# zitongbai/bipedal_control

Measured on AMD Instinct MI355X. Metric: MPC solves/s (H1, horizon=100), higher is better.
Workload: dtype f64; 1 GPU; Unitree H1 trot (template tiled from t = 0), horizon=100 intervals (dt 0.015), batch=256 per GPU perturbed initial states, cold start, 1 SQP iteration (BASELINE.json configs[1]); solver=sqp, global_batch=256, problems_on_rank0=256, shooting_nodes=108, nx=22, nu=22

## Files before the change

### bipedal_control_amd/csrc/k_node.hip

```cpp
#include <hip/hip_runtime.h>
#include <hip/hip_ext.h>

#include <stdexcept>

#include "kernel_launchers.h"
#include "launch.h"
#include "kernels/rollout.h"

namespace bpmpc {

template <int NJ>
__global__ __launch_bounds__(kWave) void k_prepare(Launch L) {
  constexpr int NX = 12 + NJ, NU = 12 + NJ;
  const int s = blockIdx.x, b = s / L.N, k = s % L.N;
  const int g = L.buf.p_grid[b];
  const int n = L.buf.g_nodes[g];
  if (k >= n) { if (threadIdx.x == 0) L.buf.n_info[s] = 0; return; }
  const size_t gs = (size_t)g * L.N + k;
  if (threadIdx.x == 0) L.buf.n_info[s] = 8 | ((L.buf.g_mode[gs] & 3) << 1) | (L.buf.g_kind[gs] == 1 ? 1 : 0);
  if (threadIdx.x < kNodeAux) {
    const int t = threadIdx.x;
    L.buf.n_aux[(size_t)s * kNodeAux + t] = t == 0 ? L.buf.g_dt[gs] : t < 5 ? L.buf.g_zref[gs * 4 + t - 1] : t < 9 ? L.buf.g_zdref[gs * 4 + t - 5] : 0.0;
  }
  prepare_node<NJ>(*L.model, L.buf.g_kind[gs], L.buf.g_mode[gs], L.buf.g_start[gs], L.cold != 0, k == n - 1, L.buf.p_tgt_n[b],
// ... 172 lines not shown
    u[(size_t)i * NU + l] = a * uff0 + (1.0 - a) * uff1 + kx;
  }
}

template <int NJ>
__global__ __launch_bounds__(kWave) void k_ls_begin(Launch L) {
  __shared__ double partial[3 * kWave + 5];
  linesearch_begin<NJ>(partial, problem_ls<NJ>(L, blockIdx.x));
}

template <int NJ>
__global__ __launch_bounds__(kWave) void k_trial(Launch L) {
  constexpr int NX = 12 + NJ, NU = 12 + NJ;
  __shared__ TrialWorkspace<NJ> ws;
  const int sidx = blockIdx.x, b = sidx / L.N, k = sidx % L.N;
  if (L.buf.done[b]) return;
  if (k >= L.buf.g_nodes[L.buf.p_grid[b]]) return;
  const NodeInputs in = node_inputs<NJ>(L, b, k);
  const double* dx = L.buf.dx + ((size_t)b * (L.N + 1) + k) * NX;
  trial_node<NJ>(*L.model, ws, in, L.buf.alpha[b], dx, L.buf.du + (size_t)sidx * NU, dx + NX, L.buf.trial_perf + (size_t)sidx * 3);
}

template <int NJ, bool CHAIN>
__global__ __launch_bounds__(kTrialWaves * kWave) __attribute__((amdgpu_waves_per_eu(3, 3)))
void k_trial_fast(Launch L) {
  using C = LinFastCfg<NJ, true, CHAIN>;
  constexpr int NX = 12 + NJ, NU = 12 + NJ, LPN = C::LPN, NPW = C::NPW;
  __shared__ LinFastNodeLds<NJ, false, CHAIN> lds[kTrialWaves * NPW];
  __shared__ LinFastShared<NJ, false> shared;
  const int sub = threadIdx.x / LPN, g = threadIdx.x % LPN;
  const int widx = blockIdx.x * (kTrialWaves * NPW) + sub;
  {
    const int total = L.batch * L.klen, w0 = blockIdx.x * (kTrialWaves * NPW), w1 = (w0 + kTrialWaves * NPW < total ? w0 + kTrialWaves * NPW : total) - 1;
    bool any = false;
    for (int pb = w0 / L.klen; pb <= w1 / L.klen; ++pb) any = any || L.buf.done[pb] == 0;
    if (!any) return;
  }
  bool valid = widx < L.batch * L.klen;
  const int b = valid ? widx / L.klen : 0, k = valid ? L.k0 + widx % L.klen : 0;
  const double* dx = L.buf.dx + ((size_t)b * (L.N + 1) + k) * NX;
  {
    const int fin = L.buf.done[b];
    const double alpha = L.buf.alpha[b];
    const int info = L.buf.n_info[(size_t)b * L.N + k];
    const size_t s0 = (size_t)b * L.N + k;
    const double* xk = L.buf.x + ((size_t)b * (L.N + 1) + k) * NX;
    const TrialPre pre = trial_preload<C>(xk, xk + NX, L.buf.u + s0 * NU, L.buf.xref + s0 * NX, dx, dx + NX, L.buf.du + s0 * NU, g, L.buf.n_aux + s0 * kNodeAux);
    load_shared_model<kTrialWaves * kWave>(*L.model, shared, threadIdx.x);
    NodeInputs in;
    in.kind = info & 1; in.mode = (info >> 1) & 3; in.dt = 0.0;
    in.x = xk; in.xnext = xk + NX; in.u = L.buf.u + s0 * NU; in.xref = L.buf.xref + s0 * NX; in.zref = nullptr; in.zdref = nullptr;
    __syncthreads();
    valid = valid && fin == 0 && info != 0;
    const size_t s = valid ? s0 : 0;
    trial_fast<NJ, C>(*L.model, shared, lds[sub], valid, in, alpha, dx, L.buf.du + s * NU, dx + NX, L.buf.trial_perf + s * 3, g, nullptr, &pre);
  }
}

template <int NJ, bool CHAIN>
__global__ __launch_bounds__(kTrialWaves * kWave) void k_constraint_values(Launch L, double* eqv) {
  using C = LinFastCfg<NJ, true, CHAIN>;
  constexpr int NX = 12 + NJ, NU = 12 + NJ, LPN = C::LPN, NPW = C::NPW;
  __shared__ LinFastNodeLds<NJ, false, CHAIN> lds[kTrialWaves * NPW];
  __shared__ LinFastShared<NJ, false> shared;
  load_shared_model<kTrialWaves * kWave>(*L.model, shared, threadIdx.x);
  __syncthreads();
  const int sub = threadIdx.x / LPN, g = threadIdx.x % LPN;
  const int widx = blockIdx.x * (kTrialWaves * NPW) + sub;
  bool valid = widx < L.batch * L.klen;
  const int b = valid ? widx / L.klen : 0, k = valid ? L.k0 + widx % L.klen : 0;
  const int grid = L.buf.p_grid[b];
  valid = valid && k < L.buf.g_nodes[grid] && L.buf.g_kind[(size_t)grid * L.N + k] == 0;
  const size_t s = valid ? (size_t)b * L.N + k : 0;
  const NodeInputs in = node_inputs<NJ>(L, b, k);
  const double* dx = L.buf.dx + ((size_t)b * (L.N + 1) + k) * NX;
  double perf[3];
  trial_fast<NJ, C, true>(*L.model, shared, lds[sub], valid, in, 0.0, dx, L.buf.du + s * NU, dx + NX, perf, g, eqv + s * kMaxEqRows);
}

template <int NJ, bool CHAIN>
__global__ __launch_bounds__(kWave) void k_rollout(const DeviceModel* model, RolloutArgs a) {
  __shared__ RolloutLds<NJ, CHAIN> w;
  load_shared_model<kWave>(*model, w.shared, threadIdx.x);
  __syncthreads();
  rollout_policy<NJ, CHAIN>(*model, w, a);
}

constexpr int kDecideThreads = 256;
template <int NJ>
__global__ __launch_bounds__(kDecideThreads) void k_ls_decide(Launch L, int look_first) {
  __shared__ double partial[3 * kDecideThreads + 5];
  linesearch_decide<NJ, kDecideThreads>(partial, problem_ls<NJ>(L, blockIdx.x), L.ls, look_first != 0);
}

constexpr int kTailThreads = 512;
template <int NJ, bool CHAIN>
__global__ __launch_bounds__(kTailThreads) void k_ls_tail(Launch L, int first_round, int max_trials, int pending) {
  using C = LinFastCfg<NJ, true, CHAIN>;
  constexpr int NX = 12 + NJ, NU = 12 + NJ, LPN = C::LPN, NPW = C::NPW, CHUNK = (kTailThreads / kWave) * NPW;
  const int b = blockIdx.x;
  if (L.buf.done[b]) return;
  __shared__ LinFastNodeLds<NJ, false, CHAIN> lds[CHUNK];
  __shared__ LinFastShared<NJ, false> shared;
  __shared__ double partial[3 * kTailThreads + 5];
  volatile const int* done = L.buf.done + b;
  volatile const double* alpha = L.buf.alpha + b;
  if (pending) {
    int bb = b;
    asm volatile("" : "+s"(bb));
    linesearch_decide<NJ, kTailThreads, true>(partial, problem_ls<NJ>(L, bb), L.ls);
    __threadfence();
    __syncthreads();
    if (*done) return;
  }
  load_shared_model<kTailThreads>(*L.model, shared, threadIdx.x);
  __syncthreads();
  const int sub = threadIdx.x / LPN, g = threadIdx.x % LPN;
  const int n = L.buf.g_nodes[L.buf.p_grid[b]];
  for (int round = first_round; round < max_trials; ++round) {
    const double al = *alpha;
    for (int k0 = 0; k0 < n; k0 += CHUNK) {
      const int k = k0 + sub;
      const bool valid = k < n;
      const int kk = valid ? k : 0;
      const size_t s = (size_t)b * L.N + kk;
      const NodeInputs in = node_inputs<NJ>(L, b, kk);
      const double* dx = L.buf.dx + ((size_t)b * (L.N + 1) + kk) * NX;
      unsigned opaque = 0;
      asm volatile("" : "+v"(opaque));
      const auto& sh = *reinterpret_cast<const LinFastShared<NJ, false>*>(reinterpret_cast<const char*>(&shared) + opaque);
      trial_fast<NJ, C>(*L.model, sh, lds[sub], valid, in, al, dx, L.buf.du + s * NU, dx + NX, L.buf.trial_perf + s * 3, g);
    }
    __threadfence();
    __syncthreads();
    int bb = b;
    asm volatile("" : "+s"(bb));
    const ProblemLS p = problem_ls<NJ>(L, bb);
    linesearch_decide<NJ, kTailThreads, false>(partial, p, L.ls);
    __threadfence();
    __syncthreads();
    if (*done) break;
  }
}

__global__ __launch_bounds__(256) void k_copy_pairs(const double* a_src, double* a_dst, size_t na, const double* b_src, double* b_dst, size_t nb,
                                                     int* iterations, int* active, int batch) {
  const size_t i0 = (size_t)blockIdx.x * blockDim.x + threadIdx.x, stride = (size_t)gridDim.x * blockDim.x;
  const double2* a2 = reinterpret_cast<const double2*>(a_src);
  const double2* b2 = reinterpret_cast<const double2*>(b_src);
  double2* ad = reinterpret_cast<double2*>(a_dst);
  double2* bd = reinterpret_cast<double2*>(b_dst);
  for (size_t i = i0; i < na / 2; i += stride) ad[i] = a2[i];
  for (size_t i = i0; i < nb / 2; i += stride) bd[i] = b2[i];
  if (i0 == 0) { if (na & 1) a_dst[na - 1] = a_src[na - 1]; if (nb & 1) b_dst[nb - 1] = b_src[nb - 1]; }
  if (iterations) for (size_t i = i0; i < (size_t)batch; i += stride) { iterations[i] = 0; active[i] = 1; }
}

namespace kl {

void prepare(int nj, int slots, hipStream_t st, const Launch& L) { KL_NJ(nj, hipLaunchKernelGGL(k_prepare<NJ>, dim3(slots), dim3(kWave), 0, st, L)); }
void linearize_reference(int nj, int slots, hipStream_t st, const Launch& L) { KL_NJ(nj, hipLaunchKernelGGL(k_linearize<NJ>, dim3(slots), dim3(kWave), 0, st, L)); }
// ... 15 lines not shown
      else launch(k_linearize_fast<NJ, false, true>);
    } else {
      if (materialise) launch(k_linearize_fast<NJ, true, false>);
      else launch(k_linearize_fast<NJ, false, false>);
    }
  });
}
void warm_shift(int nj, int slots, hipStream_t st, const Launch& L, const int* restarted) {
  KL_NJ(nj, hipLaunchKernelGGL(k_warm_shift<NJ>, dim3(slots), dim3(kWave), 0, st, L, restarted));
}
void ls_begin(int nj, int batch, hipStream_t st, const Launch& L) { KL_NJ(nj, hipLaunchKernelGGL(k_ls_begin<NJ>, dim3(batch), dim3(kWave), 0, st, L)); }
void trial_reference(int nj, int slots, hipStream_t st, const Launch& L) { KL_NJ(nj, hipLaunchKernelGGL(k_trial<NJ>, dim3(slots), dim3(kWave), 0, st, L)); }
int trial_fast_workgroups(int nj, int nodes) {
  const int per_wg = kTrialWaves * (nj == 10 ? LinFastCfg<10, true>::NPW : LinFastCfg<12, true>::NPW);
  return (nodes + per_wg - 1) / per_wg;
}
void trial_fast(int nj, int nodes, hipStream_t st, const Launch& L) {
  const int grid = trial_fast_workgroups(nj, nodes);
  KL_NJ(nj, {
    if (L.serial_legs) hipLaunchKernelGGL((k_trial_fast<NJ, true>), dim3(grid), dim3(kTrialWaves * kWave), 0, st, L);
    else hipLaunchKernelGGL((k_trial_fast<NJ, false>), dim3(grid), dim3(kTrialWaves * kWave), 0, st, L);
  });
}
void ls_decide(int nj, int batch, hipStream_t st, const Launch& L, bool look_first) { KL_NJ(nj, hipLaunchKernelGGL(k_ls_decide<NJ>, dim3(batch), dim3(kDecideThreads), 0, st, L, look_first ? 1 : 0)); }
void ls_tail(int nj, int batch, hipStream_t st, const Launch& L, int first_round, int max_trials, bool pending) {
  KL_NJ(nj, {
    if (L.serial_legs) hipLaunchKernelGGL((k_ls_tail<NJ, true>), dim3(batch), dim3(kTailThreads), 0, st, L, first_round, max_trials, pending ? 1 : 0);
    else hipLaunchKernelGGL((k_ls_tail<NJ, false>), dim3(batch), dim3(kTailThreads), 0, st, L, first_round, max_trials, pending ? 1 : 0);
  });
}
void constraint_values(int nj, int nodes, hipStream_t st, const Launch& L, double* eqv) {
  const int grid = trial_fast_workgroups(nj, nodes);
  KL_NJ(nj, {
    if (L.serial_legs) hipLaunchKernelGGL((k_constraint_values<NJ, true>), dim3(grid), dim3(kTrialWaves * kWave), 0, st, L, eqv);
    else hipLaunchKernelGGL((k_constraint_values<NJ, false>), dim3(grid), dim3(kTrialWaves * kWave), 0, st, L, eqv);
  });
}
void rollout(int nj, bool serial_legs, int batch, hipStream_t st, const DeviceModel* model, const RolloutArgs& a) {
  KL_NJ(nj, {
    constexpr bool kChainFits = LinFastCfg<NJ, false, true>::LPN == 16;
    const dim3 grid((batch + LinFastCfg<NJ>::NPW - 1) / LinFastCfg<NJ>::NPW);
    if constexpr (kChainFits) {
      if (serial_legs) { hipLaunchKernelGGL((k_rollout<NJ, true>), grid, dim3(kWave), 0, st, model, a); return; }
    }
    hipLaunchKernelGGL((k_rollout<NJ, false>), grid, dim3(kWave), 0, st, model, a);
  });
}
void copy_pairs(int grid, hipStream_t st, const double* a_src, double* a_dst, size_t na, const double* b_src, double* b_dst, size_t nb,
                int* iterations, int* active, int batch) {
  hipLaunchKernelGGL(k_copy_pairs, dim3(grid > 0 ? grid : 1), dim3(256), 0, st, a_src, a_dst, na, b_src, b_dst, nb, iterations, active, batch);
}
// ... 4 lines not shown
```

### bipedal_control_amd/csrc/kernel_launchers.h

```cpp
#pragma once
#include <hip/hip_runtime.h>

#include <cstddef>
#include <stdexcept>

namespace bpmpc {

#define KL_NJ(nj, ...)                                                          \
  do {                                                                          \
    if ((nj) == 10) { constexpr int NJ = 10; __VA_ARGS__; }                     \
    else if ((nj) == 12) { constexpr int NJ = 12; __VA_ARGS__; }                \
    else throw std::runtime_error("unsupported joint count");                   \
  } while (0)

struct Launch;
struct DeviceModel;
struct RolloutArgs;
struct DdpBuffers;
struct TickArgs;
struct TickCommandArgs;
struct RestartArgs;

namespace kl {

void prepare(int nj, int slots, hipStream_t st, const Launch& L);
void linearize_reference(int nj, int slots, hipStream_t st, const Launch& L);
void linearize_fast(int nj, bool materialise, int nodes, hipStream_t st, const Launch& L, hipEvent_t ev_start = nullptr, hipEvent_t ev_stop = nullptr);
void warm_shift(int nj, int slots, hipStream_t st, const Launch& L, const int* restarted = nullptr);
void ls_begin(int nj, int batch, hipStream_t st, const Launch& L);
void trial_reference(int nj, int slots, hipStream_t st, const Launch& L);
int trial_fast_workgroups(int nj, int nodes);
void trial_fast(int nj, int nodes, hipStream_t st, const Launch& L);
void ls_decide(int nj, int batch, hipStream_t st, const Launch& L, bool look_first = false);
void ls_tail(int nj, int batch, hipStream_t st, const Launch& L, int first_round, int max_trials, bool pending);
void constraint_values(int nj, int nodes, hipStream_t st, const Launch& L, double* eqv);
void rollout(int nj, bool serial_legs, int batch, hipStream_t st, const DeviceModel* model, const RolloutArgs& a);
void copy_pairs(int grid, hipStream_t st, const double* a_src, double* a_dst, size_t na, const double* b_src, double* b_dst, size_t nb,
                int* iterations, int* active, int batch);

void project_reference(int nj, int slots, hipStream_t st, const Launch& L);
void project_lu_s(int nj, int max_vel_rows, bool packed, int nodes, hipStream_t st, const Launch& L);
void project_fast(int nj, bool packed, bool joint_rows, int nodes, hipStream_t st, const Launch& L);

void riccati_reference(int nj, int batch, hipStream_t st, const Launch& L);
void riccati_fast(int nj, bool joint_rows, int batch, hipStream_t st, const Launch& L);
void riccati_fast8(int nj, bool joint_rows, int batch, hipStream_t st, const Launch& L);

void riccati_wave(int nj, bool two_per_simd, bool joint_rows, int batch, hipStream_t st, const Launch& L);
void riccati_rollout(int nj, int batch, hipStream_t st, const Launch& L);

void ddp_policy(int nj, int batch, hipStream_t st, const Launch& L, const DdpBuffers& d);
void ddp_cost(int nj, int batch, bool fast, hipStream_t st, const Launch& L, const DdpBuffers& d);
void ddp_select(int nj, int batch, hipStream_t st, const Launch& L, const DdpBuffers& d, double armijo);
void ddp_nominal(int nj, int batch, hipStream_t st, const Launch& L, const DdpBuffers& d);
void ddp_finish(int nj, int batch, hipStream_t st, const Launch& L, const DdpBuffers& d);
void ddp_keep_times(int batch, int N, hipStream_t st, const DdpBuffers& d, double* tp_time, int* tp_kind, int* tp_nodes, int* tp_grid);

// ... 7 lines not shown
```

### bipedal_control_amd/csrc/kernels/linesearch.h

```cpp
#pragma once
#include "node_lq.h"

namespace bpmpc {

constexpr int kMaxTargetPoints = 8;
constexpr int kStatsStride = 16;

struct LineSearchSettings {
  double g_max, g_min, alpha_decay, alpha_min, gamma_c, armijo_factor, delta_tol, cost_tol;
  int max_iterations;
};

template <int NJ>
BP_DEVICE void prepare_node(const DeviceModel& md, int kind, int mode, double t_start, bool cold, bool last, int n_pts, const double* tgt_t,
                            const double* tgt_x, const double* x0, double* xref, double* x, double* u, double* x_terminal) {
  constexpr int NX = 12 + NJ, NU = 12 + NJ;
  BP_LANES(tid, kWave) {
    if (tid < NX) {
      double val;
      if (n_pts == 1 || t_start <= tgt_t[0]) {
        val = tgt_x[tid];
      } else if (t_start >= tgt_t[n_pts - 1]) {
        val = tgt_x[(n_pts - 1) * NX + tid];
      } else {
// ... 16 lines not shown
struct TrialWorkspace {
  static constexpr int NX = 12 + NJ, NU = 12 + NJ;
  NodeWorkspace<NJ> node;
  double tx[NX], tu[NU], txn[NX];
};

template <int NJ>
BP_DEVICE void trial_node(const DeviceModel& md, TrialWorkspace<NJ>& ws, NodeInputs in, double alpha, const double* dx, const double* du,
                          const double* dxn, double* perf) {
  constexpr int NX = 12 + NJ, NU = 12 + NJ;
  BP_LANES(tid, kWave) {
    if (tid < NX) {
      ws.tx[tid] = in.x[tid] + alpha * dx[tid];
      ws.txn[tid] = in.xnext[tid] + alpha * dxn[tid];
    }
    if (tid < NU) ws.tu[tid] = (in.kind == 1) ? 0.0 : in.u[tid] + alpha * du[tid];
  }
  BP_SYNC();
  in.x = ws.tx;
  in.u = ws.tu;
  in.xnext = ws.txn;
  node_performance<NJ>(md, ws.node, in, perf);
}

struct ProblemLS {
  int n_nodes;
  const double* node_perf;
  const double* trial_perf;
  const double* x0;
  double *x, *u;
  const double *dx, *du;
  const double* summary;
  double* base;
  double* alpha;
  int* done;
  int* active;
  int* iterations;
  double* stats;
  int* remaining;
};

template <int NJ>
BP_DEVICE void linesearch_begin(double* partial , const ProblemLS& p) {
  constexpr int NX = 12 + NJ;
  BP_LANES(tid, kWave) {
    double a = 0.0, b = 0.0, c = 0.0;
    for (int k = tid; k < p.n_nodes; k += kWave) { a += p.node_perf[3 * k]; b += p.node_perf[3 * k + 1]; c += p.node_perf[3 * k + 2]; }
    if (tid < NX) { const double d = p.x0[tid] - p.x[tid]; b += d * d; }
    partial[tid] = a; partial[kWave + tid] = b; partial[2 * kWave + tid] = c;
  }
  BP_SYNC();
  BP_LANES(tid, kWave) {
    if (tid < 3) {
      double s = 0.0;
      for (int i = 0; i < kWave; ++i) s += partial[tid * kWave + i];
      partial[3 * kWave + 2 + tid] = s;
    }
  }
  BP_SYNC();
  BP_LANES(tid, kWave) {
    if (tid == 0) {
      const double a = partial[3 * kWave + 2], b = partial[3 * kWave + 3], c = partial[3 * kWave + 4];
// ... 102 lines not shown
  BP_SYNC();
  const bool accepted = partial[3 * NL] != 0.0;
  if (accepted) {
#if !defined(BPMPC_HOST_EMULATION)
#pragma unroll
    for (int j = 0; j < UPD; ++j) {
      const int idx = (int)threadIdx.x + j * NL;
      if (idx < nxe) p.x[idx] = xv[j] + alpha * dxv[j];
      if (idx < nue) p.u[idx] = uv[j] + alpha * duv[j];
    }
    int t0 = (int)threadIdx.x;
    if constexpr (!PRE) asm volatile("" : "+v"(t0));
    for (int idx = t0 + UPD * NL; idx < nxe; idx += NL) p.x[idx] += alpha * p.dx[idx];
    for (int idx = t0 + UPD * NL; idx < nue; idx += NL) p.u[idx] += alpha * p.du[idx];
#else
    BP_LANES(tid, NL) {
      for (int idx = tid; idx < (p.n_nodes + 1) * NX; idx += NL) p.x[idx] += alpha * p.dx[idx];
      for (int idx = tid; idx < p.n_nodes * NU; idx += NL) p.u[idx] += alpha * p.du[idx];
    }
#endif
  }
}

}
```

### bipedal_control_amd/csrc/kernels/riccati_fast.h

```cpp
#pragma once
#include <hip/hip_runtime.h>

#include "../device_model.h"
#include "riccati.h"
#include "project_node.h"
#include "linesearch.h"

namespace bpmpc {

struct RiccatiFastIO {
  RiccatiIO base;
  const double *Wt, *Qp, *Mt;
  const double* Vt;
  const double *lqA, *lqB, *lqb, *lqq, *lqr, *qrd, *gdt;
  const DeviceModel* model;
  const double* zero_one;
  const int* mode;
  double *Acl, *bcl;
  double *kff;
  double *mvec, *mscal;
  double* Kfull;
  double* prof;
  int k_lo, k_hi;
  double* carry;
// ... 18 lines not shown
  return __hiloint2double(hi, lo);
}
template <int NJ>
__device__ __forceinline__ void linesearch_begin_wave(double* partial , const ProblemLS& p, int lane) {
  constexpr int NX = 12 + NJ;
  {
    double a = 0.0, b = 0.0, c = 0.0;
    for (int k = lane; k < p.n_nodes; k += kWave) { a += p.node_perf[3 * k]; b += p.node_perf[3 * k + 1]; c += p.node_perf[3 * k + 2]; }
    if (lane < NX) { const double d = p.x0[lane] - p.x[lane]; b += d * d; }
    partial[lane] = a; partial[kWave + lane] = b; partial[2 * kWave + lane] = c;
  }
  lds_wave_sync();
  if (lane < 3) {
    double s = 0.0;
    for (int i = 0; i < kWave; ++i) s += partial[lane * kWave + i];
    partial[3 * kWave + 2 + lane] = s;
  }
  lds_wave_sync();
  if (lane == 0) {
    p.base[0] = partial[3 * kWave + 2]; p.base[1] = partial[3 * kWave + 3]; p.base[2] = partial[3 * kWave + 4];
    p.alpha[0] = 1.0;
    const bool run = p.active[0] != 0;
    p.done[0] = run ? 0 : 1;
    if (run) atomicAdd(p.remaining, 1);
  }
}
__device__ __forceinline__ double lds1(const double& r) {
  typedef const volatile __attribute__((address_space(3))) double* lds_cvp;
  return *(lds_cvp)(&r);
}
struct d2 { double x, y; };
__device__ __forceinline__ d2 lds_pair(const double* p) {
  const double2 v = *reinterpret_cast<const double2*>(p);
  return d2{v.x, v.y};
}

__device__ __forceinline__ double fast_reciprocal(double x) {
  double r = __builtin_amdgcn_rcp(x);
  double e = __builtin_fma(-x, r, 1.0);
  r = __builtin_fma(r, e, r);
  e = __builtin_fma(-x, r, 1.0);
  r = __builtin_fma(r, e, r);
  return r;
}

template <int ROWS>
// ... 305 lines not shown
```

### bipedal_control_amd/csrc/launch.h

```cpp
#pragma once
#include <hip/hip_runtime.h>

#include <cstddef>

#include "device_model.h"
#include "kernels/linesearch.h"
#include "kernels/node_lq.h"
#include "kernels/project_node.h"
#include "kernels/riccati_fast.h"
#include "kernels/linearize_fast.h"

namespace bpmpc {

struct Buffers {
  int *g_kind, *g_mode, *g_nodes;
  double *g_dt, *g_start, *g_zref, *g_zdref;
  int* p_grid;
  double *p_x0, *p_tgt_t, *p_tgt_x;
  int* p_tgt_n;
  double *x, *u, *x_init, *u_init, *xref;
  double *A, *B, *b, *Q, *R, *P, *q, *r, *c, *C, *D, *e, *perf;
  int* nc;
  double *Px, *Pu, *Pe, *At, *Bt, *bt, *Qt, *Rt, *Pt, *qt, *rt;
  double *Wt, *Qp, *Mt;
  double* Vt;
  int* nut;
  int* n_info;
  double* n_aux;
  double* lin_park;
  double* lin_dump;
  double* qrd;
  double *Kt, *kt, *dx, *du, *K, *summary, *dx0;
  double *Acl, *bcl, *kff, *mvec, *mscal, *rprof;
  double *x_prev, *u_prev, *K_prev, *tp_time;
  int *tp_kind, *tp_nodes, *tp_grid;
  double *roll_t, *roll_x0, *roll_x, *roll_u;
  int *roll_steps, *roll_status;
  double *g_time, *rg_t0, *rg_start, *p_t0, *p_cmd, *lib_d;
  int *rg_gait, *rg_status, *rg_rows, *lib_i;
  double* ric_carry;
  double* zero_page;
  double *trial_perf, *base, *alpha, *stats;
  int *done, *active, *iterations, *remaining;
};

struct DdpBuffers {
  int cap;
  int nv;
  double alpha_v[kMaxDdpSteps];
  double* lff;
  double *rec_t, *rec_x, *rec_u, *cost;
  int* rec_n;
  double *end_x, *end_u;
  int *roll_steps, *roll_status;
  double *sol_t, *sol_x, *sol_u;
  int* sol_n;
  double *merit0, *merit, *alpha, *update_is;
  int *accepted, *failed, *n_points;
};

constexpr int kLinMaxEvents = 8;
struct Launch {
  const DeviceModel* model;
  Buffers buf;
  int batch, N;
  int k0, klen;
// ... 45 lines not shown
}

template <int NJ>
__device__ __forceinline__ ProblemLS problem_ls(const Launch& L, int b) {
  constexpr int NX = 12 + NJ, NU = 12 + NJ;
  ProblemLS p;
  const size_t s0 = (size_t)b * L.N;
  p.n_nodes = L.buf.g_nodes[L.buf.p_grid[b]];
  p.node_perf = L.buf.perf + s0 * 3;
  p.trial_perf = L.buf.trial_perf + s0 * 3;
  p.x0 = L.buf.p_x0 + (size_t)b * NX;
  p.x = L.buf.x + (size_t)b * (L.N + 1) * NX;
  p.u = L.buf.u + s0 * NU;
  p.dx = L.buf.dx + (size_t)b * (L.N + 1) * NX;
  p.du = L.buf.du + s0 * NU;
  p.summary = L.buf.summary + (size_t)b * 4;
  p.base = L.buf.base + (size_t)b * 3;
  p.alpha = L.buf.alpha + b;
  p.done = L.buf.done + b;
  p.active = L.buf.active + b;
  p.iterations = L.buf.iterations + b;
  p.stats = L.buf.stats + (size_t)b * kStatsStride;
  p.remaining = L.buf.remaining;
  return p;
}

template <int NJ>
__device__ __forceinline__ bool riccati_fast_io(const Launch& L, RiccatiFastIO& io, double* lds_scratch ) {
  constexpr int NX = 12 + NJ, NU = 12 + NJ;
  const int b = blockIdx.x;
  const int tid_ = threadIdx.x;
  io.with_ls = L.k0 == 0;
  if (io.with_ls) io.ls = problem_ls<NJ>(L, b);
  if (!L.buf.active[b]) {
    if (io.with_ls && tid_ < kWave) linesearch_begin_wave<NJ>(lds_scratch, io.ls, tid_);
    return false;
  }
  const size_t s0 = (size_t)b * L.N;
  double* dx0 = L.buf.dx0 + (size_t)b * NX;
  if (tid_ < NX) dx0[tid_] = L.buf.p_x0[(size_t)b * NX + tid_] - L.buf.x[(size_t)b * (L.N + 1) * NX + tid_];
  __syncthreads();
  io.base.N = L.buf.g_nodes[L.buf.p_grid[b]];
  io.base.nut = L.buf.nut + s0;
  io.base.At = L.buf.At + s0 * NX * NX; io.base.Bt = L.buf.Bt + s0 * NX * NU; io.base.bt = L.buf.bt + s0 * NX;
  io.base.Qt = L.buf.Qt + s0 * NX * NX; io.base.Rt = L.buf.Rt + s0 * NU * NU; io.base.Pt = L.buf.Pt + s0 * NU * NX;
  io.base.qt = L.buf.qt + s0 * NX; io.base.rt = L.buf.rt + s0 * NU;
// ... 26 lines not shown
```

### bipedal_control_amd/csrc/solver.hip

```cpp
#include <hip/hip_runtime.h>

#include <cmath>
#include <cstdint>
#include <algorithm>
#include <cstring>
#include <map>
#include <tuple>
#include <memory>
#include <stdexcept>
#include <string>
#include <vector>

#include "solver.h"
#include "reference_gen.h"
#include "kernels/rollout.h"

#define TIMED_ON(on, cls, ...)                                                      \
  do {                                                                              \
    hipEvent_t ev_a_, ev_b_;                                                        \
    time_begin(cls, &ev_a_, &ev_b_, on);                                            \
    __VA_ARGS__;                                                                    \
    time_end(cls, ev_a_, ev_b_, on);                                                \
    HIP_CHECK(hipGetLastError());                                                   \
  } while (0)
// ... 38 lines not shown
  if (sweep_eight_waves()) { TIMED("riccati", kl::riccati_fast8(nj(), !sweep_completes_joint_rows(), batch, stream, L)); return; }
  if (!sweep_wave_regime()) {
    TIMED("riccati", kl::riccati_fast(nj(), !sweep_completes_joint_rows(), batch, stream, L));
    return;
  }
  TIMED("riccati", { kl::riccati_wave(nj(), sweep_two_per_simd(), !sweep_completes_joint_rows(), batch, stream, L); if (L.k0 == 0) kl::riccati_rollout(nj(), batch, stream, L); });
}
void bpmpc_solver::stage_riccati() {
  const Launch L = launch_params();
  if (settings.reference_kernels) TIMED("riccati", kl::riccati_reference(nj(), batch, stream, L));
  else launch_riccati(L);
}
void bpmpc_solver::stage_linesearch() {
  const Launch L = launch_params();
  if (settings.reference_kernels) HIP_CHECK(hipMemsetAsync(buf.remaining, 0, sizeof(int), stream));
  hipEvent_t ev_a, ev_b;
  time_begin("linesearch", &ev_a, &ev_b);
  if (settings.reference_kernels) kl::ls_begin(nj(), batch, stream, L);
  int max_trials = 0;
  for (double a = 1.0; a >= ls.alpha_min; a *= ls.alpha_decay) ++max_trials;
  if (!settings.reference_kernels) {
    const int nodes = batch * L.klen;
    static const int wide_rounds = [] { const char* e = std::getenv("BPMPC_LS_WIDE_ROUNDS"); const int v = e ? std::atoi(e) : 2; return v < 1 ? 1 : v; }();
    int round = 0;
    bool pending = false;
    for (; round < wide_rounds && round < max_trials; ++round) {
      kl::trial_fast(nj(), nodes, stream, L);
      pending = round > 0 && (round + 1 == wide_rounds || round + 1 == max_trials);
      if (!pending) kl::ls_decide(nj(), batch, stream, L, round > 0);
    }
    kl::ls_tail(nj(), batch, stream, L, round, max_trials, pending);
    HIP_CHECK(hipGetLastError());
    time_end("linesearch", ev_a, ev_b);
    return;
  }
  for (int t = 0; t < max_trials; ++t) {
    kl::trial_reference(nj(), batch * settings.max_nodes, stream, L);
    kl::ls_decide(nj(), batch, stream, L);
    HIP_CHECK(hipGetLastError());
    HIP_CHECK(hipMemcpyAsync(h_remaining, buf.remaining, sizeof(int), hipMemcpyDeviceToHost, stream));
    HIP_CHECK(hipStreamSynchronize(stream));
    if (*h_remaining <= 0) break;
  }
  time_end("linesearch", ev_a, ev_b);
}
void bpmpc_solver::pipelined_backward() {
  const int chunks = settings.pipeline_chunks;
  const int n = n_nodes_max;
  HIP_CHECK(hipEventRecord(ev_go, stream));
  HIP_CHECK(hipStreamWaitEvent(producer_stream, ev_go, 0));
  for (int c = 0; c < chunks; ++c) {
    const int hi = n - (int)((long long)n * c / chunks), lo = n - (int)((long long)n * (c + 1) / chunks);
    if (hi <= lo) continue;
    Launch L = launch_params();
// ... 106 lines not shown
  b.n_info = s->alloc<int>("n_info", S, true);
  b.n_aux = s->alloc<double>("n_aux", S * kNodeAux);
  b.At = b.Bt = b.bt = b.Qt = b.Rt = b.Pt = b.qt = b.rt = b.Kt = b.kt = b.Wt = b.Qp = b.Mt = b.Vt = nullptr;
  if (s->settings.reference_kernels) {
    b.At = s->alloc<double>("At", S * NX * NX); b.Bt = s->alloc<double>("Bt", S * NX * NU); b.bt = s->alloc<double>("bt", S * NX);
    b.Qt = s->alloc<double>("Qt", S * NX * NX); b.Rt = s->alloc<double>("Rt", S * NU * NU); b.Pt = s->alloc<double>("Pt", S * NU * NX);
    b.qt = s->alloc<double>("qt", S * NX); b.rt = s->alloc<double>("rt", S * NU);
    b.Kt = s->alloc<double>("Kt", S * NU * NX); b.kt = s->alloc<double>("kt", S * NU);
  } else {
    const size_t wp = ((NX + 1 + NU + 15) / 16) * 16;
    b.Wt = s->alloc<double>("Wt", S * NX * wp); b.Qp = s->alloc<double>("Qp", S * NX * 32); b.Mt = s->alloc<double>("Mt", S * NU * wp);
    b.Vt = s->alloc<double>("Vt", S * (NX - 12) * wp);
  }
  b.dx = s->alloc<double>("dx", B * (N + 1) * NX); b.du = s->alloc<double>("du", S * NU);
  b.K = s->alloc<double>("K", S * NU * NX);
  b.Acl = s->alloc<double>("Acl", S * NX * NX); b.bcl = s->alloc<double>(nullptr, S * NX); b.kff = s->alloc<double>(nullptr, S * NU);
  b.mvec = s->alloc<double>(nullptr, S * NX); b.mscal = s->alloc<double>(nullptr, S);
  b.rprof = s->alloc<double>("rprof", std::max<size_t>(B * 8, 32768));
  b.summary = s->alloc<double>("summary", B * 4); b.dx0 = s->alloc<double>(nullptr, B * NX);
  b.trial_perf = s->alloc<double>("trial_perf", S * 3); b.base = s->alloc<double>("base", B * 3); b.alpha = s->alloc<double>("alpha", B);
  b.stats = s->alloc<double>("stats", B * kStatsStride);
  b.done = s->alloc<int>("done", B, true); b.active = s->alloc<int>("active", B, true); b.iterations = s->alloc<int>("iterations", B, true);
  b.remaining = s->alloc<int>(nullptr, 1);
  {
    const size_t tick = B * (64 + NX * 8 + N * 4 + (N + 1) * 8 + 64) + (size_t)kRefLibCapacity * 16 + 4096;
    const size_t solution = (B * ((N + 1) * NX + N * NU + N * NU * NX + kStatsStride)) * sizeof(double) + 4096;
    s->xfer_cap = std::max(tick, std::min<size_t>(size_t(1) << 20, solution));
    s->xfer = s->alloc<char>(nullptr, s->xfer_cap);
  }
  if (s->is_ddp()) {
    DdpBuffers& d = s->ddp;
    d.cap = (int)N + 1;
    {
      constexpr double kContractionRate = 0.5;
      d.nv = 0; d.alpha_v[d.nv++] = 0.0;
      for (double al = s->rm.ddp.ls_max_step_length; al >= s->rm.ddp.ls_min_step_length && d.nv < kMaxDdpSteps; al *= kContractionRate) d.alpha_v[d.nv++] = al;
    }
    const size_t P = B * (size_t)d.cap, V = (size_t)d.nv;
    d.lff = s->alloc<double>("ddp_lff", S * NU);
    d.rec_t = s->alloc<double>(nullptr, V * P); d.rec_x = s->alloc<double>(nullptr, V * P * NX); d.rec_u = s->alloc<double>(nullptr, V * P * NU); d.rec_n = s->alloc<int>("ddp_rec_n", V * B, true);
    d.cost = s->alloc<double>(nullptr, V * P * 3);
    d.end_x = s->alloc<double>(nullptr, V * B * NX); d.end_u = s->alloc<double>(nullptr, V * B * NU); d.roll_steps = s->alloc<int>("ddp_roll_steps", V * B * 2, true); d.roll_status = s->alloc<int>("ddp_roll_status", V * B, true);
    d.sol_t = s->alloc<double>("ddp_t", P); d.sol_x = s->alloc<double>(nullptr, P * NX); d.sol_u = s->alloc<double>("ddp_u", P * NU); d.sol_n = s->alloc<int>(nullptr, B);
    d.merit0 = s->alloc<double>(nullptr, B); d.merit = s->alloc<double>(nullptr, B); d.alpha = s->alloc<double>(nullptr, B);
    d.update_is = s->alloc<double>("ddp_update_is", B);
    d.accepted = s->alloc<int>(nullptr, B); d.failed = s->alloc<int>(nullptr, B); d.n_points = s->alloc<int>("ddp_points", B, true);
// ... 769 lines not shown
```

Measured before the change: 350,100 solves/s.

## Compact second line-search trial round to a list of still-open problems

After the first line-search decision, problems that reject the full step are appended to a small device-side open list, and the second trial round launches workgroups only for those listed problems instead of every node of the batch. The decide step is also split into a request phase that preloads x, dx, u and du into registers and a finish phase that does the reduction and the update. The aim is to cut wasted trial workgroups and hide global-memory latency in the decide kernel. Problems that overflow the 32-slot list fall back to the per-problem tail kernel, which adds branching and atomics and raises register pressure.

```diff
diff --git a/bipedal_control_amd/csrc/k_node.hip b/bipedal_control_amd/csrc/k_node.hip
--- a/bipedal_control_amd/csrc/k_node.hip
+++ b/bipedal_control_amd/csrc/k_node.hip
@@ -218,10 +218,31 @@
 }
 
 template <int NJ, bool CHAIN>
+__device__ __forceinline__ void trial_fast_group(const Launch& L, LinFastNodeLds<NJ, false, CHAIN>& node_lds, LinFastShared<NJ, false>& shared, bool valid, int b, int k, int g) {
+  using C = LinFastCfg<NJ, true, CHAIN>;
+  constexpr int NX = 12 + NJ, NU = 12 + NJ;
+  const double* dx = L.buf.dx + ((size_t)b * (L.N + 1) + k) * NX;
+  const int fin = L.buf.done[b];
+  const double alpha = L.buf.alpha[b];
+  const int info = L.buf.n_info[(size_t)b * L.N + k];
+  const size_t s0 = (size_t)b * L.N + k;
+  const double* xk = L.buf.x + ((size_t)b * (L.N + 1) + k) * NX;
+  const TrialPre pre = trial_preload<C>(xk, xk + NX, L.buf.u + s0 * NU, L.buf.xref + s0 * NX, dx, dx + NX, L.buf.du + s0 * NU, g, L.buf.n_aux + s0 * kNodeAux);
+  load_shared_model<kTrialWaves * kWave>(*L.model, shared, threadIdx.x);
+  NodeInputs in;
+  in.kind = info & 1; in.mode = (info >> 1) & 3; in.dt = 0.0;
+  in.x = xk; in.xnext = xk + NX; in.u = L.buf.u + s0 * NU; in.xref = L.buf.xref + s0 * NX; in.zref = nullptr; in.zdref = nullptr;
+  __syncthreads();
+  valid = valid && fin == 0 && info != 0;
+  const size_t s = valid ? s0 : 0;
+  trial_fast<NJ, C>(*L.model, shared, node_lds, valid, in, alpha, dx, L.buf.du + s * NU, dx + NX, L.buf.trial_perf + s * 3, g, nullptr, &pre);
+}
+
+template <int NJ, bool CHAIN>
 __global__ __launch_bounds__(kTrialWaves * kWave) __attribute__((amdgpu_waves_per_eu(3, 3)))
 void k_trial_fast(Launch L) {
   using C = LinFastCfg<NJ, true, CHAIN>;
-  constexpr int NX = 12 + NJ, NU = 12 + NJ, LPN = C::LPN, NPW = C::NPW;
+  constexpr int LPN = C::LPN, NPW = C::NPW;
   __shared__ LinFastNodeLds<NJ, false, CHAIN> lds[kTrialWaves * NPW];
   __shared__ LinFastShared<NJ, false> shared;
   const int sub = threadIdx.x / LPN, g = threadIdx.x % LPN;
@@ -232,25 +253,25 @@
     for (int pb = w0 / L.klen; pb <= w1 / L.klen; ++pb) any = any || L.buf.done[pb] == 0;
     if (!any) return;
   }
-  bool valid = widx < L.batch * L.klen;
+  const bool valid = widx < L.batch * L.klen;
   const int b = valid ? widx / L.klen : 0, k = valid ? L.k0 + widx % L.klen : 0;
-  const double* dx = L.buf.dx + ((size_t)b * (L.N + 1) + k) * NX;
-  {
-    const int fin = L.buf.done[b];
-    const double alpha = L.buf.alpha[b];
-    const int info = L.buf.n_info[(size_t)b * L.N + k];
-    const size_t s0 = (size_t)b * L.N + k;
-    const double* xk = L.buf.x + ((size_t)b * (L.N + 1) + k) * NX;
-    const TrialPre pre = trial_preload<C>(xk, xk + NX, L.buf.u + s0 * NU, L.buf.xref + s0 * NX, dx, dx + NX, L.buf.du + s0 * NU, g, L.buf.n_aux + s0 * kNodeAux);
-    load_shared_model<kTrialWaves * kWave>(*L.model, shared, threadIdx.x);
-    NodeInputs in;
-    in.kind = info & 1; in.mode = (info >> 1) & 3; in.dt = 0.0;
-    in.x = xk; in.xnext = xk + NX; in.u = L.buf.u + s0 * NU; in.xref = L.buf.xref + s0 * NX; in.zref = nullptr; in.zdref = nullptr;
-    __syncthreads();
-    valid = valid && fin == 0 && info != 0;
-    const size_t s = valid ? s0 : 0;
-    trial_fast<NJ, C>(*L.model, shared, lds[sub], valid, in, alpha, dx, L.buf.du + s * NU, dx + NX, L.buf.trial_perf + s * 3, g, nullptr, &pre);
-  }
+  trial_fast_group<NJ, CHAIN>(L, lds[sub], shared, valid, b, k, g);
+}
+
+template <int NJ, bool CHAIN>
+__global__ __launch_bounds__(kTrialWaves * kWave) __attribute__((amdgpu_waves_per_eu(3, 3)))
+void k_trial_list(Launch L, int wgs_per_problem) {
+  using C = LinFastCfg<NJ, true, CHAIN>;
+  constexpr int LPN = C::LPN, NPW = C::NPW;
+  __shared__ LinFastNodeLds<NJ, false, CHAIN> lds[kTrialWaves * NPW];
+  __shared__ LinFastShared<NJ, false> shared;
+  const int slot = blockIdx.x / wgs_per_problem, chunk = blockIdx.x % wgs_per_problem;
+  if (slot >= L.buf.ls_open_count[0]) return;
+  const int b = L.buf.ls_open_list[slot];
+  const int sub = threadIdx.x / LPN, g = threadIdx.x % LPN;
+  const int j = chunk * (kTrialWaves * NPW) + sub;
+  const bool valid = j < L.klen;
+  trial_fast_group<NJ, CHAIN>(L, lds[sub], shared, valid, b, valid ? L.k0 + j : 0, g);
 }
 
 template <int NJ, bool CHAIN>
@@ -284,9 +305,18 @@
 
 constexpr int kDecideThreads = 256;
 template <int NJ>
-__global__ __launch_bounds__(kDecideThreads) void k_ls_decide(Launch L, int look_first) {
+__global__ __launch_bounds__(kDecideThreads) void k_ls_decide_ref(Launch L) {
   __shared__ double partial[3 * kDecideThreads + 5];
-  linesearch_decide<NJ, kDecideThreads>(partial, problem_ls<NJ>(L, blockIdx.x), L.ls, look_first != 0);
+  linesearch_decide<NJ, kDecideThreads>(partial, problem_ls<NJ>(L, blockIdx.x), L.ls);
+}
+template <int NJ>
+__global__ __launch_bounds__(kDecideThreads) void k_ls_decide(Launch L, int look_first, int append) {
+  __shared__ double partial[3 * kDecideThreads + 5];
+  if (look_first && L.buf.done[blockIdx.x]) return;
+  const ProblemLS p = problem_ls<NJ>(L, blockIdx.x);
+  DecidePre<NJ, kDecideThreads, true> q;
+  linesearch_decide_request<NJ, kDecideThreads, true>(q, p);
+  linesearch_decide_finish<NJ, kDecideThreads, true>(partial, q, p, L.ls, append != 0);
 }
 
 constexpr int kTailThreads = 512;
@@ -304,13 +334,24 @@
   if (pending) {
     int bb = b;
     asm volatile("" : "+s"(bb));
-    linesearch_decide<NJ, kTailThreads, true>(partial, problem_ls<NJ>(L, bb), L.ls);
-    __threadfence();
+    const ProblemLS p = problem_ls<NJ>(L, bb);
+    const int slot = pending == 2 ? p.open_slot[0] : 0;
+    DecidePre<NJ, kTailThreads, true> q;
+    linesearch_decide_request<NJ, kTailThreads, true>(q, p);
+    load_shared_model<kTailThreads>(*L.model, shared, threadIdx.x);
+    if (slot < kLsOpenCap) {
+      linesearch_decide_finish<NJ, kTailThreads, true>(partial, q, p, L.ls, false);
+      __threadfence();
+      __syncthreads();
+      if (*done) return;
+    } else {
+      first_round -= 1;
+      __syncthreads();
+    }
+  } else {
+    load_shared_model<kTailThreads>(*L.model, shared, threadIdx.x);
     __syncthreads();
-    if (*done) return;
-  }
-  load_shared_model<kTailThreads>(*L.model, shared, threadIdx.x);
-  __syncthreads();
+  }
   const int sub = threadIdx.x / LPN, g = threadIdx.x % LPN;
   const int n = L.buf.g_nodes[L.buf.p_grid[b]];
   for (int round = first_round; round < max_trials; ++round) {
@@ -332,7 +373,9 @@
     int bb = b;
     asm volatile("" : "+s"(bb));
     const ProblemLS p = problem_ls<NJ>(L, bb);
-    linesearch_decide<NJ, kTailThreads, false>(partial, p, L.ls);
+    DecidePre<NJ, kTailThreads, false> q;
+    linesearch_decide_request<NJ, kTailThreads, false>(q, p);
+    linesearch_decide_finish<NJ, kTailThreads, false>(partial, q, p, L.ls, false);
     __threadfence();
     __syncthreads();
     if (*done) break;
@@ -394,11 +437,21 @@
     else hipLaunchKernelGGL((k_trial_fast<NJ, false>), dim3(grid), dim3(kTrialWaves * kWave), 0, st, L);
   });
 }
-void ls_decide(int nj, int batch, hipStream_t st, const Launch& L, bool look_first) { KL_NJ(nj, hipLaunchKernelGGL(k_ls_decide<NJ>, dim3(batch), dim3(kDecideThreads), 0, st, L, look_first ? 1 : 0)); }
-void ls_tail(int nj, int batch, hipStream_t st, const Launch& L, int first_round, int max_trials, bool pending) {
-  KL_NJ(nj, {
-    if (L.serial_legs) hipLaunchKernelGGL((k_ls_tail<NJ, true>), dim3(batch), dim3(kTailThreads), 0, st, L, first_round, max_trials, pending ? 1 : 0);
-    else hipLaunchKernelGGL((k_ls_tail<NJ, false>), dim3(batch), dim3(kTailThreads), 0, st, L, first_round, max_trials, pending ? 1 : 0);
+void trial_list(int nj, int batch, hipStream_t st, const Launch& L) {
+  const int per_problem = trial_fast_workgroups(nj, L.klen), grid = (batch < kLsOpenCap ? batch : kLsOpenCap) * per_problem;
+  KL_NJ(nj, {
+    if (L.serial_legs) hipLaunchKernelGGL((k_trial_list<NJ, true>), dim3(grid), dim3(kTrialWaves * kWave), 0, st, L, per_problem);
+    else hipLaunchKernelGGL((k_trial_list<NJ, false>), dim3(grid), dim3(kTrialWaves * kWave), 0, st, L, per_problem);
+  });
+}
+void ls_decide(int nj, int batch, hipStream_t st, const Launch& L) { KL_NJ(nj, hipLaunchKernelGGL(k_ls_decide_ref<NJ>, dim3(batch), dim3(kDecideThreads), 0, st, L)); }
+void ls_decide_fast(int nj, int batch, hipStream_t st, const Launch& L, bool look_first, bool append) {
+  KL_NJ(nj, hipLaunchKernelGGL(k_ls_decide<NJ>, dim3(batch), dim3(kDecideThreads), 0, st, L, look_first ? 1 : 0, append ? 1 : 0));
+}
+void ls_tail(int nj, int batch, hipStream_t st, const Launch& L, int first_round, int max_trials, int pending) {
+  KL_NJ(nj, {
+    if (L.serial_legs) hipLaunchKernelGGL((k_ls_tail<NJ, true>), dim3(batch), dim3(kTailThreads), 0, st, L, first_round, max_trials, pending);
+    else hipLaunchKernelGGL((k_ls_tail<NJ, false>), dim3(batch), dim3(kTailThreads), 0, st, L, first_round, max_trials, pending);
   });
 }
 void constraint_values(int nj, int nodes, hipStream_t st, const Launch& L, double* eqv) {
diff --git a/bipedal_control_amd/csrc/kernel_launchers.h b/bipedal_control_amd/csrc/kernel_launchers.h
--- a/bipedal_control_amd/csrc/kernel_launchers.h
+++ b/bipedal_control_amd/csrc/kernel_launchers.h
@@ -31,8 +31,10 @@
 void trial_reference(int nj, int slots, hipStream_t st, const Launch& L);
 int trial_fast_workgroups(int nj, int nodes);
 void trial_fast(int nj, int nodes, hipStream_t st, const Launch& L);
-void ls_decide(int nj, int batch, hipStream_t st, const Launch& L, bool look_first = false);
-void ls_tail(int nj, int batch, hipStream_t st, const Launch& L, int first_round, int max_trials, bool pending);
+void trial_list(int nj, int batch, hipStream_t st, const Launch& L);
+void ls_decide(int nj, int batch, hipStream_t st, const Launch& L);
+void ls_decide_fast(int nj, int batch, hipStream_t st, const Launch& L, bool look_first, bool append);
+void ls_tail(int nj, int batch, hipStream_t st, const Launch& L, int first_round, int max_trials, int pending);
 void constraint_values(int nj, int nodes, hipStream_t st, const Launch& L, double* eqv);
 void rollout(int nj, bool serial_legs, int batch, hipStream_t st, const DeviceModel* model, const RolloutArgs& a);
 void copy_pairs(int grid, hipStream_t st, const double* a_src, double* a_dst, size_t na, const double* b_src, double* b_dst, size_t nb,
diff --git a/bipedal_control_amd/csrc/kernels/linesearch.h b/bipedal_control_amd/csrc/kernels/linesearch.h
--- a/bipedal_control_amd/csrc/kernels/linesearch.h
+++ b/bipedal_control_amd/csrc/kernels/linesearch.h
@@ -62,6 +62,8 @@
   in.xnext = ws.txn;
   node_performance<NJ>(md, ws.node, in, perf);
 }
+
+constexpr int kLsOpenCap = 32;
 
 struct ProblemLS {
   int n_nodes;
@@ -78,6 +80,11 @@
   int* iterations;
   double* stats;
   int* remaining;
+  int index;
+  int n_alloc;
+  int* open_count;
+  int* open_list;
+  int* open_slot;
 };
 
 template <int NJ>
@@ -226,4 +233,151 @@
   }
 }
 
-}
+#if !defined(BPMPC_HOST_EMULATION)
+template <int NJ, int NL, bool PRE>
+struct DecidePre {
+  static constexpr int UPD = PRE ? (2400 + NL - 1) / NL : 0;
+  double xv[UPD + 1], dxv[UPD + 1], uv[UPD + 1], duv[UPD + 1];
+  double tp[3];
+  double hx0, hx, hdx;
+  double alpha, base[3], summary[4];
+  int done, iterations;
+};
+
+template <int NJ, int NL, bool PRE>
+__device__ __forceinline__ void linesearch_decide_request(DecidePre<NJ, NL, PRE>& q, const ProblemLS& p) {
+  constexpr int NX = 12 + NJ, NU = 12 + NJ, UPD = DecidePre<NJ, NL, PRE>::UPD;
+  const int tid = (int)threadIdx.x;
+  q.done = p.done[0];
+  q.alpha = p.alpha[0];
+  q.iterations = p.iterations[0];
+#pragma unroll
+  for (int j = 0; j < 3; ++j) q.base[j] = p.base[j];
+#pragma unroll
+  for (int j = 0; j < 4; ++j) q.summary[j] = p.summary[j];
+  const int kt = tid < p.n_alloc ? tid : 0, kh = tid < NX ? tid : 0;
+#pragma unroll
+  for (int j = 0; j < 3; ++j) q.tp[j] = p.trial_perf[3 * kt + j];
+  q.hx0 = p.x0[kh]; q.hx = p.x[kh]; q.hdx = p.dx[kh];
+  const int nxa = (p.n_alloc + 1) * NX, nua = p.n_alloc * NU;
+#pragma unroll
+  for (int j = 0; j < UPD; ++j) {
+    const int idx = tid + j * NL;
+    const int ix = idx < nxa ? idx : 0, iu = idx < nua ? idx : 0;
+    q.xv[j] = p.x[ix]; q.dxv[j] = p.dx[ix]; q.uv[j] = p.u[iu]; q.duv[j] = p.du[iu];
+  }
+}
+
+template <int NJ, int NL, bool PRE>
+__device__ __forceinline__ void linesearch_decide_finish(double* partial , const DecidePre<NJ, NL, PRE>& q, const ProblemLS& p,
+                                                         const LineSearchSettings& st, bool append) {
+  constexpr int NX = 12 + NJ, NU = 12 + NJ, UPD = DecidePre<NJ, NL, PRE>::UPD;
+  constexpr int NSUM = NL < 256 ? NL : 256;
+  constexpr int UB = 16;
+  static_assert(NSUM >= 2 * UB, "the first two batches of the sums lie inside a row");
+  if (q.done) return;
+  const int tid = (int)threadIdx.x;
+  const int n_nodes = p.n_nodes;
+  const double alpha = q.alpha;
+  {
+    double a = 0.0, b = 0.0, c = 0.0;
+    if (tid < NSUM) {
+      if (tid < n_nodes) { a += q.tp[0]; b += q.tp[1]; c += q.tp[2]; }
+      int k1 = tid + NSUM;
+      if constexpr (!PRE) asm volatile("" : "+v"(k1));
+      for (int k = k1; k < n_nodes; k += NSUM) { a += p.trial_perf[3 * k]; b += p.trial_perf[3 * k + 1]; c += p.trial_perf[3 * k + 2]; }
+    }
+    if (tid < NX) { const double d = q.hx0 - (q.hx + alpha * q.hdx); b += d * d; }
+    partial[tid] = a; partial[NL + tid] = b; partial[2 * NL + tid] = c;
+  }
+  __syncthreads();
+  if (tid < 3) {
+    int lim = n_nodes > NX ? n_nodes : NX;
+    if (lim > NSUM) lim = NSUM;
+    const double* row = partial + tid * NL;
+    double s = 0.0, v[UB], w[UB];
+#pragma unroll
+    for (int j = 0; j < UB; ++j) v[j] = row[j];
+    for (int i = 0; i < lim; i += UB) {
+#pragma unroll
+      for (int j = 0; j < UB; ++j) { const int nx_ = i + UB + j; w[j] = row[nx_ < NSUM ? nx_ : NSUM - 1]; }
+#pragma unroll
+      for (int j = 0; j < UB; ++j) if (i + j < lim) s += v[j];
+#pragma unroll
+      for (int j = 0; j < UB; ++j) v[j] = w[j];
+    }
+    partial[3 * NL + 2 + tid] = s;
+  }
+  __syncthreads();
+  if (tid == 0) {
+    const double merit = partial[3 * NL + 2], dyn = partial[3 * NL + 3], eq = partial[3 * NL + 4];
+    const double merit0 = q.base[0];
+    const double viol0 = sqrt(q.base[1] + q.base[2]);
+    const double viol = sqrt(dyn + eq);
+    const double descent = alpha * q.summary[0];
+    double gamma_c = st.gamma_c;
+    if constexpr (!PRE) asm volatile("" : "+v"(gamma_c));
+    bool accepted;
+    if (viol > st.g_max) {
+      accepted = viol < (1.0 - gamma_c) * viol0;
+    } else if (viol < st.g_min && viol0 < st.g_min && descent < 0.0) {
+      accepted = merit < merit0 + st.armijo_factor * descent;
+    } else {
+      accepted = merit < (merit0 - gamma_c * viol0) || viol < (1.0 - gamma_c) * viol0;
+    }
+    const bool numerical = q.summary[3] != 0.0;
+    if (numerical) accepted = false;
+    const double next_alpha = alpha * st.alpha_decay;
+    const bool tiny = next_alpha * sqrt(q.summary[1]) < st.delta_tol && next_alpha * sqrt(q.summary[2]) < st.delta_tol;
+    const bool give_up = !accepted && (numerical || tiny || !(next_alpha >= st.alpha_min));
+    partial[3 * NL] = accepted ? 1.0 : 0.0;
+    partial[3 * NL + 1] = give_up ? 1.0 : 0.0;
+    if (accepted || give_up) {
+      double* s = p.stats;
+      const int it = q.iterations + 1;
+      p.iterations[0] = it;
+      const double dxn = accepted ? alpha * sqrt(q.summary[1]) : 0.0, dun = accepted ? alpha * sqrt(q.summary[2]) : 0.0;
+      const double s6 = accepted ? merit : merit0, s7 = accepted ? dyn : q.base[1], s8 = accepted ? eq : q.base[2], s9 = accepted ? alpha : 0.0;
+      s[0] = (double)n_nodes;
+      s[1] = (double)it;
+      s[2] = numerical ? 2.0 : (accepted ? 0.0 : 1.0);
+      s[3] = merit0; s[4] = q.base[1]; s[5] = q.base[2];
+      s[6] = s6; s[7] = s7; s[8] = s8;
+      s[9] = s9;
+      s[10] = q.summary[0];
+      s[11] = dxn; s[12] = dun;
+      bool keep_going = it < st.max_iterations;
+      if (keep_going && s9 < st.alpha_min) keep_going = false;
+      if (keep_going && fabs(s6 - merit0) < st.cost_tol && sqrt(s7 + s8) < st.g_min) keep_going = false;
+      if (keep_going && dxn < st.delta_tol && dun < st.delta_tol) keep_going = false;
+      p.active[0] = keep_going ? 1 : 0;
+      p.done[0] = 1;
+      atomicSub(p.remaining, 1);
+    } else {
+      p.alpha[0] = next_alpha;
+      if (append) {
+        const int slot = atomicAdd(p.open_count, 1);
+        p.open_slot[0] = slot;
+        if (slot < kLsOpenCap) p.open_list[slot] = p.index;
+      }
+    }
+  }
+  __syncthreads();
+  const bool accepted = partial[3 * NL] != 0.0;
+  if (accepted) {
+    const int nxe = (n_nodes + 1) * NX, nue = n_nodes * NU;
+#pragma unroll
+    for (int j = 0; j < UPD; ++j) {
+      const int idx = tid + j * NL;
+      if (idx < nxe) p.x[idx] = q.xv[j] + alpha * q.dxv[j];
+      if (idx < nue) p.u[idx] = q.uv[j] + alpha * q.duv[j];
+    }
+    int t0 = tid;
+    if constexpr (!PRE) asm volatile("" : "+v"(t0));
+    for (int idx = t0 + UPD * NL; idx < nxe; idx += NL) p.x[idx] += alpha * p.dx[idx];
+    for (int idx = t0 + UPD * NL; idx < nue; idx += NL) p.u[idx] += alpha * p.du[idx];
+  }
+}
+#endif
+
+}
diff --git a/bipedal_control_amd/csrc/kernels/riccati_fast.h b/bipedal_control_amd/csrc/kernels/riccati_fast.h
--- a/bipedal_control_amd/csrc/kernels/riccati_fast.h
+++ b/bipedal_control_amd/csrc/kernels/riccati_fast.h
@@ -64,6 +64,7 @@
     p.alpha[0] = 1.0;
     const bool run = p.active[0] != 0;
     p.done[0] = run ? 0 : 1;
+    p.open_count[0] = 0;
     if (run) atomicAdd(p.remaining, 1);
   }
 }
diff --git a/bipedal_control_amd/csrc/launch.h b/bipedal_control_amd/csrc/launch.h
--- a/bipedal_control_amd/csrc/launch.h
+++ b/bipedal_control_amd/csrc/launch.h
@@ -42,6 +42,7 @@
   double* zero_page;
   double *trial_perf, *base, *alpha, *stats;
   int *done, *active, *iterations, *remaining;
+  int *ls_open_count, *ls_open_list, *ls_open_slot;
 };
 
 struct DdpBuffers {
@@ -133,6 +134,11 @@
   p.iterations = L.buf.iterations + b;
   p.stats = L.buf.stats + (size_t)b * kStatsStride;
   p.remaining = L.buf.remaining;
+  p.index = b;
+  p.n_alloc = L.N;
+  p.open_count = L.buf.ls_open_count;
+  p.open_list = L.buf.ls_open_list;
+  p.open_slot = L.buf.ls_open_slot + b;
   return p;
 }
 
diff --git a/bipedal_control_amd/csrc/solver.hip b/bipedal_control_amd/csrc/solver.hip
--- a/bipedal_control_amd/csrc/solver.hip
+++ b/bipedal_control_amd/csrc/solver.hip
@@ -84,14 +84,16 @@
   if (!settings.reference_kernels) {
     const int nodes = batch * L.klen;
     static const int wide_rounds = [] { const char* e = std::getenv("BPMPC_LS_WIDE_ROUNDS"); const int v = e ? std::atoi(e) : 2; return v < 1 ? 1 : v; }();
+    const bool listed = wide_rounds == 2;
     int round = 0;
     bool pending = false;
     for (; round < wide_rounds && round < max_trials; ++round) {
-      kl::trial_fast(nj(), nodes, stream, L);
+      if (round > 0 && listed) kl::trial_list(nj(), batch, stream, L);
+      else kl::trial_fast(nj(), nodes, stream, L);
       pending = round > 0 && (round + 1 == wide_rounds || round + 1 == max_trials);
-      if (!pending) kl::ls_decide(nj(), batch, stream, L, round > 0);
-    }
-    kl::ls_tail(nj(), batch, stream, L, round, max_trials, pending);
+      if (!pending) kl::ls_decide_fast(nj(), batch, stream, L, round > 0, listed && round == 0 && max_trials > 1);
+    }
+    kl::ls_tail(nj(), batch, stream, L, round, max_trials, pending ? (listed ? 2 : 1) : 0);
     HIP_CHECK(hipGetLastError());
     time_end("linesearch", ev_a, ev_b);
     return;
@@ -244,6 +246,7 @@
   b.stats = s->alloc<double>("stats", B * kStatsStride);
   b.done = s->alloc<int>("done", B, true); b.active = s->alloc<int>("active", B, true); b.iterations = s->alloc<int>("iterations", B, true);
   b.remaining = s->alloc<int>(nullptr, 1);
+  b.ls_open_count = s->alloc<int>(nullptr, 1); b.ls_open_list = s->alloc<int>(nullptr, kLsOpenCap); b.ls_open_slot = s->alloc<int>(nullptr, B);
   {
     const size_t tick = B * (64 + NX * 8 + N * 4 + (N + 1) * 8 + 64) + (size_t)kRefLibCapacity * 16 + 4096;
     const size_t solution = (B * ((N + 1) * NX + N * NU + N * NU * NX + kStatsStride)) * sizeof(double) + 4096;
```

Result: no change. 347,100 solves/s (-0.8%).
